# bing164/PL-VI-ORBSLAM3

Measured on AMD Instinct MI355X. Metric: frames/sec ORB+LSD extract+match, 640×480 mono, 1/2/4/8 MI355X, higher is better.
Workload: dtype u8; 1 GPU; C1+C2+C3: ORB extract (1000 feats, 1.2, 8 levels, FAST 20/7) || LSD+LBD (200 lines, scale 0.8, 2 octaves) as one HIP-stream schedule, then ORB kNN-2 + LineMatcher::match vs previous frame; batch=3072, width=640, height=480, parallelism=sequence-sharded x1, gather=False, inflight=2

## Files before the change

pl-vi-orbslam3_amd/csrc/match.hip:

```cpp
#include <hip/hip_runtime.h>

#include <climits>
#include <cstring>
#include <mutex>
#include <algorithm>
#include <vector>

#include "plvi_common.h"

namespace plvi {

constexpr int kKnnQ = 256;
constexpr int kKnnChunk = 256;

__global__ __launch_bounds__(256) void hamming_knn2_kernel(const uint8_t* __restrict__ q, const int* __restrict__ nq,
                                                           int nq_cap, const uint8_t* __restrict__ t,
                                                           const int* __restrict__ nt, int nt_cap,
                                                           int* __restrict__ idx0, int* __restrict__ d0o,
                                                           int* __restrict__ idx1, int* __restrict__ d1o) {
    __shared__ uint4 tr[kKnnChunk * 2];
    const int pair = blockIdx.y;
    const int nQ = min(nq[pair], nq_cap), nT = min(nt[pair], nt_cap);
    const int qi = blockIdx.x * kKnnQ + threadIdx.x;
    if (blockIdx.x * kKnnQ >= nQ) return;
    const bool active = qi < nQ;
    uint32_t a[8];
    {
        const uint4* qp = reinterpret_cast<const uint4*>(q + ((size_t)pair * nq_cap + (active ? qi : 0)) * 32);
        const uint4 x = qp[0], y = qp[1];
        a[0] = x.x; a[1] = x.y; a[2] = x.z; a[3] = x.w; a[4] = y.x; a[5] = y.y; a[6] = y.z; a[7] = y.w;
    }
    int b0 = INT_MAX, b1 = INT_MAX, j0 = -1, j1 = -1;
    const uint4* tp = reinterpret_cast<const uint4*>(t + (size_t)pair * nt_cap * 32);
    for (int base = 0; base < nT; base += kKnnChunk) {
        const int n = min(kKnnChunk, nT - base);
        __syncthreads();
        for (int i = threadIdx.x; i < n * 2; i += 256) tr[i] = tp[(size_t)base * 2 + i];
        __syncthreads();
        for (int j = 0; j < n; ++j) {
            const uint4 x = tr[2 * j], y = tr[2 * j + 1];
            int d = __popc(a[0] ^ x.x) + __popc(a[1] ^ x.y) + __popc(a[2] ^ x.z) + __popc(a[3] ^ x.w) +
                    __popc(a[4] ^ y.x) + __popc(a[5] ^ y.y) + __popc(a[6] ^ y.z) + __popc(a[7] ^ y.w);
            if (d < b1) {
                if (d < b0) {
                    b1 = b0; j1 = j0; b0 = d; j0 = base + j;
                } else {
                    b1 = d; j1 = base + j;
                }
            }
        }
    }
    if (active) {
        const size_t o = (size_t)pair * nq_cap + qi;
        idx0[o] = j0; d0o[o] = b0; idx1[o] = j1; d1o[o] = b1;
    }
}

__global__ __launch_bounds__(256) void line_match_finish_kernel(const int* __restrict__ n1, const int* __restrict__ n2,
                                                                int cap1, int cap2, const int* __restrict__ i0_12,
                                                                const int* __restrict__ d0_12,
                                                                const int* __restrict__ d1_12,
                                                                const int* __restrict__ i0_21,
                                                                const int* __restrict__ d0_21,
                                                                const int* __restrict__ d1_21, float nnr,
                                                                int* __restrict__ m12, int* __restrict__ nmatch) {
    __shared__ int s_cnt;
    const int p = blockIdx.x;
    const int a = min(n1[p], cap1), b = min(n2[p], cap2);
    if (threadIdx.x == 0) s_cnt = 0;
    __syncthreads();
    int local = 0;
    for (int i = threadIdx.x; i < a; i += 256) {
        const size_t o = (size_t)p * cap1 + i;
        int m = -1;
        if (b >= 2 && (float)d0_12[o] < (float)d1_12[o] * nnr) m = i0_12[o];
        if (m >= 0) {
            const size_t q = (size_t)p * cap2 + m;
            const int back = (a >= 2 && (float)d0_21[q] < (float)d1_21[q] * nnr) ? i0_21[q] : -1;
            if (back != i) m = -1;
        }
        m12[o] = m;
        local += m >= 0;
    }
    atomicAdd(&s_cnt, local);
    __syncthreads();
    if (threadIdx.x == 0) nmatch[p] = s_cnt;
}

int launch_knn2(const uint8_t* d_q, const int* d_nq, int nq_cap, const uint8_t* d_t, const int* d_nt, int nt_cap,
                int n_pairs, int* i0, int* d0, int* i1, int* d1, hipStream_t st) {
    if (n_pairs <= 0 || nq_cap <= 0) return PLVI_OK;
    dim3 grid((nq_cap + kKnnQ - 1) / kKnnQ, n_pairs);
    hipLaunchKernelGGL(hamming_knn2_kernel, grid, dim3(256), 0, st, d_q, d_nq, nq_cap, d_t, d_nt, nt_cap, i0, d0, i1,
                       d1);
    PLVI_CHECK(hipGetLastError());
    return PLVI_OK;
}

struct MatchCtx {
    std::mutex mu;
    DevBuf q, t, cnt, out;
    size_t qcap = 0, tcap = 0;
    hipStream_t st = nullptr;
    int ensure(size_t nq, size_t nt) {
        if (!st) PLVI_CHECK(hipStreamCreateWithFlags(&st, hipStreamNonBlocking));
        if (nq > qcap) {
            q.~DevBuf(); new (&q) DevBuf();
            out.~DevBuf(); new (&out) DevBuf();
            if (q.alloc(nq * 32) || out.alloc(nq * 4 * sizeof(int))) return PLVI_E_HIP;
            qcap = nq;
        }
        if (nt > tcap) {
            t.~DevBuf(); new (&t) DevBuf();
            if (t.alloc(nt * 32)) return PLVI_E_HIP;
            tcap = nt;
        }
        if (!cnt.p && cnt.alloc(2 * sizeof(int))) return PLVI_E_HIP;
        return PLVI_OK;
    }
};
static MatchCtx g_match;

int knn2_host(const uint8_t* q, int nq, const uint8_t* t, int nt, int* i0, int* d0, int* i1, int* d1) {
    if (nq < 0 || nt < 0 || (nq && !q) || (nt && !t)) return PLVI_E_BADARG;
    if (nq == 0) return PLVI_OK;
    std::lock_guard<std::mutex> lk(g_match.mu);
    int rc = g_match.ensure((size_t)nq, (size_t)std::max(nt, 1));
    if (rc) return rc;
    hipStream_t st = g_match.st;
    int counts[2] = {nq, nt};
    PLVI_CHECK(hipMemcpyAsync(g_match.q.p, q, (size_t)nq * 32, hipMemcpyHostToDevice, st));
    if (nt) PLVI_CHECK(hipMemcpyAsync(g_match.t.p, t, (size_t)nt * 32, hipMemcpyHostToDevice, st));
    PLVI_CHECK(hipMemcpyAsync(g_match.cnt.p, counts, sizeof(counts), hipMemcpyHostToDevice, st));
    int* o = g_match.out.as<int>();
    rc = launch_knn2(g_match.q.as<uint8_t>(), g_match.cnt.as<int>(), nq, g_match.t.as<uint8_t>(),
                     g_match.cnt.as<int>() + 1, std::max(nt, 1), 1, o, o + nq, o + 2 * nq, o + 3 * nq, st);
    if (rc) return rc;
    std::vector<int> h((size_t)4 * nq);
    PLVI_CHECK(hipMemcpyAsync(h.data(), o, h.size() * sizeof(int), hipMemcpyDeviceToHost, st));
    PLVI_CHECK(hipStreamSynchronize(st));
    for (int i = 0; i < nq; ++i) {
        if (i0) i0[i] = h[i];
        if (d0) d0[i] = h[nq + i];
        if (i1) i1[i] = h[2 * nq + i];
        if (d1) d1[i] = h[3 * nq + i];
    }
    return PLVI_OK;
}

}

extern "C" int plvi_hamming_knn2_batch(const uint8_t* d_q, const int* d_nq, int nq_cap, const uint8_t* d_t,
                                       const int* d_nt, int nt_cap, int n_pairs, int* d_idx0, int* d_d0, int* d_idx1,
                                       int* d_d1, void* stream) {
    if (!d_q || !d_t || !d_nq || !d_nt || nq_cap < 0 || nt_cap < 0 || n_pairs < 0) return PLVI_E_BADARG;
    return plvi::launch_knn2(d_q, d_nq, nq_cap, d_t, d_nt, nt_cap, n_pairs, d_idx0, d_d0, d_idx1, d_d1,
                             (hipStream_t)stream);
}

extern "C" int plvi_line_match_batch(const uint8_t* d_desc1, const int* d_n1, int cap1, const uint8_t* d_desc2,
                                     const int* d_n2, int cap2, int n_pairs, float nnr, int* d_scratch,
                                     int* d_matches_12, int* d_nmatch, void* stream) {
    if (!d_desc1 || !d_desc2 || !d_n1 || !d_n2 || !d_scratch || !d_matches_12 || !d_nmatch || n_pairs < 0)
        return PLVI_E_BADARG;
    if (n_pairs == 0) return PLVI_OK;
    hipStream_t st = (hipStream_t)stream;
    int* s = d_scratch;
    int *i0a = s, *d0a = s + (size_t)n_pairs * cap1, *i1a = s + 2 * (size_t)n_pairs * cap1,
        *d1a = s + 3 * (size_t)n_pairs * cap1;
    int* t = s + 4 * (size_t)n_pairs * cap1;
    int *i0b = t, *d0b = t + (size_t)n_pairs * cap2, *i1b = t + 2 * (size_t)n_pairs * cap2,
        *d1b = t + 3 * (size_t)n_pairs * cap2;
    int rc = plvi::launch_knn2(d_desc1, d_n1, cap1, d_desc2, d_n2, cap2, n_pairs, i0a, d0a, i1a, d1a, st);
    if (rc) return rc;
    rc = plvi::launch_knn2(d_desc2, d_n2, cap2, d_desc1, d_n1, cap1, n_pairs, i0b, d0b, i1b, d1b, st);
    if (rc) return rc;
    hipLaunchKernelGGL(plvi::line_match_finish_kernel, dim3(n_pairs), dim3(256), 0, st, d_n1, d_n2, cap1, cap2, i0a,
                       d0a, d1a, i0b, d0b, d1b, nnr, d_matches_12, d_nmatch);
    PLVI_CHECK(hipGetLastError());
    return PLVI_OK;
}

extern "C" int plvi_hamming_knn2(const uint8_t* q, int nq, const uint8_t* t, int nt, int* idx0, int* d0, int* idx1,
                                 int* d1) {
    return plvi::knn2_host(q, nq, t, nt, idx0, d0, idx1, d1);
}

extern "C" int plvi_line_match_nnr_inout(const uint8_t* desc1, int n1, const uint8_t* desc2, int n2, float nnr,
                                         int* matches_12, int n_prev) {
    if (n1 < 0 || n2 < 0 || n_prev < 0 || (n1 > 0 && !matches_12)) return PLVI_E_BADARG;
    if (n1 > 0 && n2 < 2) return PLVI_E_BADARG;
    std::vector<int> i0(n1), d0(n1), i1(n1), d1(n1);
    int rc = plvi::knn2_host(desc1, n1, desc2, n2, i0.data(), d0.data(), i1.data(), d1.data());
    if (rc) return rc;
    for (int i = n_prev; i < n1; ++i) matches_12[i] = -1;
    int matches = 0;
    for (int i = 0; i < n1; ++i) {
        if ((float)d0[i] < (float)d1[i] * nnr) {
            matches_12[i] = i0[i];
            ++matches;
        }
    }
    return matches;
}

extern "C" int plvi_line_match_nnr(const uint8_t* desc1, int n1, const uint8_t* desc2, int n2, float nnr,
                                   int* matches_12) {
    return plvi_line_match_nnr_inout(desc1, n1, desc2, n2, nnr, matches_12, 0);
}

extern "C" int plvi_line_match_inout(const uint8_t* desc1, int n1, const uint8_t* desc2, int n2, float nnr,
                                     int* matches_12, int n_prev) {
    if (n1 < 0 || n2 < 0 || n_prev < 0 || (n1 > 0 && !matches_12)) return PLVI_E_BADARG;
    std::vector<int> m21(n2 > 0 ? n2 : 1);
    std::vector<int> keep(matches_12, matches_12 + std::min(n_prev, n1));
    int matches = plvi_line_match_nnr_inout(desc1, n1, desc2, n2, nnr, matches_12, n_prev);
    if (matches < 0) return matches;
    int rc = plvi_line_match_nnr(desc2, n2, desc1, n1, nnr, m21.data());
    if (rc < 0) return rc;
    for (int i1 = 0; i1 < n1; ++i1)
        if (matches_12[i1] >= n2) {
            std::copy(keep.begin(), keep.end(), matches_12);
            return PLVI_E_BADARG;
        }
    for (int i1 = 0; i1 < n1; ++i1) {
        int& i2 = matches_12[i1];
        if (i2 >= 0 && m21[i2] != i1) {
            i2 = -1;
            --matches;
        }
    }
    return matches;
}

extern "C" int plvi_line_match(const uint8_t* desc1, int n1, const uint8_t* desc2, int n2, float nnr,
                               int* matches_12) {
    return plvi_line_match_inout(desc1, n1, desc2, n2, nnr, matches_12, 0);
}

namespace plvi {
__global__ __launch_bounds__(256) void descriptor_distance_kernel(const uint8_t* __restrict__ a,
                                                                  const uint8_t* __restrict__ b, int n, int shift,
                                                                  int* __restrict__ out) {
    const int i = blockIdx.x * 256 + threadIdx.x;
    if (i >= n) return;
    const uint4* pa = reinterpret_cast<const uint4*>(a + (size_t)i * 32);
    const uint4* pb = reinterpret_cast<const uint4*>(b + (size_t)i * 32);
    const uint4 a0 = pa[0], a1 = pa[1], b0 = pb[0], b1 = pb[1];
    const unsigned w[8] = {a0.x ^ b0.x, a0.y ^ b0.y, a0.z ^ b0.z, a0.w ^ b0.w,
                           a1.x ^ b1.x, a1.y ^ b1.y, a1.z ^ b1.z, a1.w ^ b1.w};
    int d = 0;
#pragma unroll
    for (int k = 0; k < 8; ++k) d += (int)((unsigned)__popc(w[k]) >> (shift - 24));
    out[i] = d;
}
}

extern "C" int plvi_descriptor_distance_batch(const uint8_t* d_a, const uint8_t* d_b, int n, int line_matcher_quirk,
                                              int* d_out, void* stream) {
    if (n < 0 || (n && (!d_a || !d_b || !d_out))) return PLVI_E_BADARG;
    if (n == 0) return PLVI_OK;
    hipLaunchKernelGGL(plvi::descriptor_distance_kernel, dim3((n + 255) / 256), dim3(256), 0, (hipStream_t)stream,
                       d_a, d_b, n, line_matcher_quirk ? 25 : 24, d_out);
    PLVI_CHECK(hipGetLastError());
    return PLVI_OK;
}
```

Measured before the change: 59920 frames/s.

## Compute Hamming kNN-2 with i8 MFMA tiles and fuse line matching

Replaces the scalar popcount Hamming kNN-2 with a kernel that bit-expands descriptors into int8 vectors and computes distances with 16x16x64 i8 MFMA instructions. Distance and train index are packed into a single sortable key so top-2 selection uses med3/min. Train chunks are staged in LDS in an MFMA-friendly layout. Line matching now runs as one fused kernel per pair that does both directions plus the ratio and cross check in LDS, which removes two launches and the global scratch traffic. The old paths remain behind an environment or compile flag and a size cap. The bit-packed key encoding and the MFMA expansion add correctness risk.

Result: faster. 61290 frames/s (median of 6 runs) (+2.3%).

```diff
diff --git a/pl-vi-orbslam3_amd/csrc/match.hip b/pl-vi-orbslam3_amd/csrc/match.hip
--- a/pl-vi-orbslam3_amd/csrc/match.hip
+++ b/pl-vi-orbslam3_amd/csrc/match.hip
@@ -1,11 +1,13 @@
 #include <hip/hip_runtime.h>
 
 #include <climits>
+#include <cstdlib>
 #include <cstring>
 #include <mutex>
 #include <algorithm>
 #include <vector>
 
+#include "match_tile.h"
 #include "plvi_common.h"
 
 namespace plvi {
@@ -87,12 +89,191 @@
     if (threadIdx.x == 0) nmatch[p] = s_cnt;
 }
 
+typedef int v4i __attribute__((ext_vector_type(4)));
+constexpr int kTileQ = 4;
+constexpr int kLdsPieces = kKnnChunk * 4;
+
+__device__ __forceinline__ void stage_train_chunk(uint2* lds, const uint4* tp, int base, int nT) {
+    for (int i = threadIdx.x; i < kKnnChunk * 2; i += 256) {
+        const int row = i >> 1, h = i & 1;
+        uint4 v = make_uint4(0, 0, 0, 0);
+        if (base + row < nT) v = tp[(size_t)base * 2 + i];
+        uint2* d = lds + (row >> 4) * 64 + h * 32 + (row & 15);
+        d[0] = make_uint2(v.x, v.y);
+        d[16] = make_uint2(v.z, v.w);
+    }
+}
+
+template <bool kMask>
+__device__ __forceinline__ void knn2_tile(const v4i (&qa)[kTileQ][4], uint2 w, int j0, int nT, int (&b0)[kTileQ],
+                                          int (&b1)[kTileQ]) {
+    uint32_t e[16];
+    expand_train_word(w.x, e);
+    expand_train_word(w.y, e + 8);
+    v4i a[4];
+#pragma unroll
+    for (int m = 0; m < 4; ++m) a[m] = v4i{(int)e[4 * m], (int)e[4 * m + 1], (int)e[4 * m + 2], (int)e[4 * m + 3]};
+#pragma unroll
+    for (int qt = 0; qt < kTileQ; ++qt) {
+        v4i acc = {0, 0, 0, 0};
+#pragma unroll
+        for (int m = 0; m < 4; ++m) acc = __builtin_amdgcn_mfma_i32_16x16x64_i8(a[m], qa[qt][m], acc, 0, 0, 0);
+#pragma unroll
+        for (int r = 0; r < 4; ++r) {
+            int k = make_key(acc[r], j0 + r);
+            if (kMask) k = j0 + r < nT ? k : kKeySentinel;
+            top2_update(b0[qt], b1[qt], k);
+        }
+    }
+}
+
+__device__ __forceinline__ void knn2_sweep(const uint8_t* __restrict__ qtab, int nQ, int q0,
+                                           const uint8_t* __restrict__ ttab, int nT, uint2* lds, int& k0, int& k1,
+                                           int& popq) {
+    const int lane = threadIdx.x & 63, c = lane & 15, g = lane >> 4;
+    const int qw = q0 + (threadIdx.x >> 6) * 64;
+    const bool waveActive = qw < nQ;
+    v4i qa[kTileQ][4];
+    int b0[kTileQ], b1[kTileQ], pq[kTileQ];
+#pragma unroll
+    for (int qt = 0; qt < kTileQ; ++qt) {
+        const int qi = qw + qt * 16 + c;
+        uint2 w = make_uint2(0, 0);
+        if (qi < nQ) w = *reinterpret_cast<const uint2*>(qtab + (size_t)qi * 32 + 8 * g);
+        uint32_t e[16];
+        expand_query_word(w.x, e);
+        expand_query_word(w.y, e + 8);
+#pragma unroll
+        for (int m = 0; m < 4; ++m)
+            qa[qt][m] = v4i{(int)e[4 * m], (int)e[4 * m + 1], (int)e[4 * m + 2], (int)e[4 * m + 3]};
+        pq[qt] = popc32(w.x) + popc32(w.y);
+        b0[qt] = b1[qt] = kKeySentinel;
+    }
+    const uint4* tp = reinterpret_cast<const uint4*>(ttab);
+    for (int base = 0; base < nT; base += kKnnChunk) {
+        __syncthreads();
+        stage_train_chunk(lds, tp, base, nT);
+        __syncthreads();
+        if (!waveActive) continue;
+        const int n = min(kKnnChunk, nT - base);
+        const int full = n >> 4;
+        for (int tl = 0; tl < full; ++tl)
+            knn2_tile<false>(qa, lds[tl * 64 + lane], base + tl * 16 + 4 * g, nT, b0, b1);
+        if (n & 15) knn2_tile<true>(qa, lds[full * 64 + lane], base + full * 16 + 4 * g, nT, b0, b1);
+    }
+    k0 = k1 = kKeySentinel;
+    popq = 0;
+#pragma unroll
+    for (int qt = 0; qt < kTileQ; ++qt) {
+#pragma unroll
+        for (int x = 16; x <= 32; x <<= 1) {
+            const int p0 = __shfl_xor(b0[qt], x), p1 = __shfl_xor(b1[qt], x);
+            top2_merge(b0[qt], b1[qt], p0, p1);
+            pq[qt] += __shfl_xor(pq[qt], x);
+        }
+        if (qt == g) {
+            k0 = b0[qt];
+            k1 = b1[qt];
+            popq = pq[qt];
+        }
+    }
+}
+
+__global__ __launch_bounds__(256, 2) void hamming_knn2_mfma_kernel(const uint8_t* __restrict__ q,
+                                                                const int* __restrict__ nq, int nq_cap,
+                                                                const uint8_t* __restrict__ t,
+                                                                const int* __restrict__ nt, int nt_cap,
+                                                                int* __restrict__ idx0, int* __restrict__ d0o,
+                                                                int* __restrict__ idx1, int* __restrict__ d1o) {
+    __shared__ uint2 lds[kLdsPieces];
+    const int pair = blockIdx.y;
+    const int nQ = min(nq[pair], nq_cap), nT = min(nt[pair], nt_cap);
+    const int q0 = blockIdx.x * kKnnQ;
+    if (q0 >= nQ) return;
+    int k0, k1, popq;
+    knn2_sweep(q + (size_t)pair * nq_cap * 32, nQ, q0, t + (size_t)pair * nt_cap * 32, nT, lds, k0, k1, popq);
+    const int qi = q0 + threadIdx.x;
+    if (qi < nQ) {
+        const size_t o = (size_t)pair * nq_cap + qi;
+        int j0, j1, e0, e1;
+        decode_key(k0, popq, j0, e0);
+        decode_key(k1, popq, j1, e1);
+        idx0[o] = j0; d0o[o] = e0; idx1[o] = j1; d1o[o] = e1;
+    }
+}
+
+__global__ __launch_bounds__(256, 2) void line_match_fused_kernel(const uint8_t* __restrict__ desc1,
+                                                               const int* __restrict__ n1, int cap1,
+                                                               const uint8_t* __restrict__ desc2,
+                                                               const int* __restrict__ n2, int cap2, float nnr,
+                                                               int* __restrict__ m12, int* __restrict__ nmatch) {
+    extern __shared__ uint2 lm_lds[];
+    __shared__ int s_cnt;
+    int* fwd = reinterpret_cast<int*>(lm_lds + kLdsPieces);
+    int* back = fwd + cap1;
+    const int p = blockIdx.x;
+    const int a = min(n1[p], cap1), b = min(n2[p], cap2);
+    const uint8_t* t1 = desc1 + (size_t)p * cap1 * 32;
+    const uint8_t* t2 = desc2 + (size_t)p * cap2 * 32;
+    if (threadIdx.x == 0) s_cnt = 0;
+    const bool both = a >= 2 && b >= 2;
+    if (both) {
+        for (int q0 = 0; q0 < a; q0 += kKnnQ) {
+            int k0, k1, popq;
+            knn2_sweep(t1, a, q0, t2, b, lm_lds, k0, k1, popq);
+            const int qi = q0 + threadIdx.x;
+            if (qi < a) {
+                int j0, j1, e0, e1;
+                decode_key(k0, popq, j0, e0);
+                decode_key(k1, popq, j1, e1);
+                fwd[qi] = (float)e0 < (float)e1 * nnr ? j0 : -1;
+            }
+        }
+        for (int q0 = 0; q0 < b; q0 += kKnnQ) {
+            int k0, k1, popq;
+            knn2_sweep(t2, b, q0, t1, a, lm_lds, k0, k1, popq);
+            const int qi = q0 + threadIdx.x;
+            if (qi < b) {
+                int j0, j1, e0, e1;
+                decode_key(k0, popq, j0, e0);
+                decode_key(k1, popq, j1, e1);
+                back[qi] = (float)e0 < (float)e1 * nnr ? j0 : -1;
+            }
+        }
+    }
+    __syncthreads();
+    int local = 0;
+    for (int i = threadIdx.x; i < a; i += 256) {
+        int m = both ? fwd[i] : -1;
+        if (m >= 0 && back[m] != i) m = -1;
+        m12[(size_t)p * cap1 + i] = m;
+        local += m >= 0;
+    }
+    if (local) atomicAdd(&s_cnt, local);
+    __syncthreads();
+    if (threadIdx.x == 0) nmatch[p] = s_cnt;
+}
+
+#ifndef PLVI_MATCH_MFMA
+#define PLVI_MATCH_MFMA 1
+#endif
+constexpr int kLineFusedCap = 1024;
+
+static bool match_mfma_enabled() {
+    const char* e = getenv("PLVI_MATCH_MFMA");
+    return e && *e ? atoi(e) != 0 : PLVI_MATCH_MFMA != 0;
+}
+
 int launch_knn2(const uint8_t* d_q, const int* d_nq, int nq_cap, const uint8_t* d_t, const int* d_nt, int nt_cap,
                 int n_pairs, int* i0, int* d0, int* i1, int* d1, hipStream_t st) {
     if (n_pairs <= 0 || nq_cap <= 0) return PLVI_OK;
     dim3 grid((nq_cap + kKnnQ - 1) / kKnnQ, n_pairs);
-    hipLaunchKernelGGL(hamming_knn2_kernel, grid, dim3(256), 0, st, d_q, d_nq, nq_cap, d_t, d_nt, nt_cap, i0, d0, i1,
-                       d1);
+    if (nt_cap <= kKeyMaxTrain && match_mfma_enabled())
+        hipLaunchKernelGGL(hamming_knn2_mfma_kernel, grid, dim3(256), 0, st, d_q, d_nq, nq_cap, d_t, d_nt, nt_cap, i0,
+                           d0, i1, d1);
+    else
+        hipLaunchKernelGGL(hamming_knn2_kernel, grid, dim3(256), 0, st, d_q, d_nq, nq_cap, d_t, d_nt, nt_cap, i0, d0,
+                           i1, d1);
     PLVI_CHECK(hipGetLastError());
     return PLVI_OK;
 }
@@ -165,6 +346,13 @@
         return PLVI_E_BADARG;
     if (n_pairs == 0) return PLVI_OK;
     hipStream_t st = (hipStream_t)stream;
+    if (cap1 <= plvi::kLineFusedCap && cap2 <= plvi::kLineFusedCap && plvi::match_mfma_enabled()) {
+        const size_t lds = plvi::kLdsPieces * sizeof(uint2) + (size_t)(std::max(cap1, 0) + std::max(cap2, 0)) * 4;
+        hipLaunchKernelGGL(plvi::line_match_fused_kernel, dim3(n_pairs), dim3(256), lds, st, d_desc1, d_n1, cap1,
+                           d_desc2, d_n2, cap2, nnr, d_matches_12, d_nmatch);
+        PLVI_CHECK(hipGetLastError());
+        return PLVI_OK;
+    }
     int* s = d_scratch;
     int *i0a = s, *d0a = s + (size_t)n_pairs * cap1, *i1a = s + 2 * (size_t)n_pairs * cap1,
         *d1a = s + 3 * (size_t)n_pairs * cap1;
diff --git a/pl-vi-orbslam3_amd/csrc/match_tile.h b/pl-vi-orbslam3_amd/csrc/match_tile.h
--- /dev/null
+++ b/pl-vi-orbslam3_amd/csrc/match_tile.h
@@ -0,0 +1,69 @@
+#pragma once
+#include <stdint.h>
+
+#ifndef PLVI_HD
+#ifdef __HIPCC__
+#define PLVI_HD __host__ __device__ __forceinline__
+#else
+#define PLVI_HD static inline
+#endif
+#endif
+
+namespace plvi {
+
+constexpr int kKeySentinel = 0x7fffffff;
+constexpr int kKeyMaxTrain = 65535;
+
+PLVI_HD void expand_train_word(uint32_t w, uint32_t out[8]) {
+#pragma unroll
+    for (int j = 0; j < 7; ++j) out[j] = w & (0x01010101u << j);
+    out[7] = (w >> 7) & 0x01010101u;
+}
+
+PLVI_HD void expand_query_word(uint32_t w, uint32_t out[8]) {
+#pragma unroll
+    for (int j = 0; j < 8; ++j) {
+        const uint32_t mag = j < 7 ? (64u >> j) : 64u;
+        out[j] = mag * 0x01010101u + ((w >> j) & 0x01010101u) * (256u - 2u * mag);
+    }
+}
+
+PLVI_HD int popc32(uint32_t w) { return __builtin_popcount(w); }
+
+PLVI_HD int make_key(int acc, int j) { return (int)(((uint32_t)acc << 10) | (uint32_t)j); }
+
+PLVI_HD int imin(int a, int b) { return a < b ? a : b; }
+PLVI_HD int imax(int a, int b) { return a > b ? a : b; }
+PLVI_HD int imed3(int a, int b, int c) {
+#if defined(__HIP_DEVICE_COMPILE__)
+    int r;
+    asm("v_med3_i32 %0, %1, %2, %3" : "=v"(r) : "v"(a), "v"(b), "v"(c));
+    return r;
+#else
+    return imax(imin(a, b), imin(imax(a, b), c));
+#endif
+}
+
+PLVI_HD void top2_update(int& b0, int& b1, int k) {
+    b1 = imed3(b0, b1, k);
+    b0 = imin(b0, k);
+}
+
+PLVI_HD void top2_merge(int& b0, int& b1, int p0, int p1) {
+    const int hi = imax(b0, p0);
+    b0 = imin(b0, p0);
+    b1 = imin(hi, imin(b1, p1));
+}
+
+PLVI_HD void decode_key(int key, int popq, int& idx, int& dist) {
+    if (key == kKeySentinel) {
+        idx = -1;
+        dist = 0x7fffffff;
+    } else {
+        key += popq << 16;
+        idx = key & 0xffff;
+        dist = key >> 16;
+    }
+}
+
+}
```
